# zju3dv/OnePose_Plus_Plus

Measured on AMD Instinct MI355X. Metric: query images/sec (2D-3D match fwd) at 512x512 img x 5k pts, higher is better.
Workload: dtype f32 (operands as exact bf16 triples, f32 accumulate)

## Files before the change

### onepose_plus_plus_amd/csrc/enc_layer64.hip

```cpp
#include <stdlib.h>

#include <type_traits>

#include "enc_frag.h"

namespace {

constexpr int R64 = 64, C = 256, NW = 8, NT = 512, D = 32;
constexpr int SA = a_stride_bytes(C);
constexpr int SS = C + 4;
constexpr int OFF_S = R64 * SA, OFF_Z = OFF_S + 32 * SS * 4;
constexpr size_t kLds64 = OFF_Z + 1024;

__global__ __launch_bounds__(NT) void enc_layer64_kernel(const OppEncChain a) {
  extern __shared__ __attribute__((aligned(16))) char smem[];
  char* A = smem;
  float* S = reinterpret_cast<float*>(smem + OFF_S);
  float* z_sh = reinterpret_cast<float*>(smem + OFF_Z);

  const int tid = threadIdx.x, lane = tid & 63;
  const int wave = __builtin_amdgcn_readfirstlane(tid >> 6);
  const int half = lane >> 5, l31 = lane & 31;

  const int chunks0 = (a.len0 + R64 - 1) / R64;
  const int stream = (int)blockIdx.x >= chunks0 ? 1 : 0;
  const int cidx = stream ? blockIdx.x - chunks0 : blockIdx.x;
  const int seg_len = stream ? a.len1 : a.len0;
  const int row0 = (stream ? a.len0 : 0) + cidx * R64;
  const int nrows = min(R64, seg_len - cidx * R64);
  const float* qrows = (stream && a.q1 != nullptr) ? a.q1 + (size_t)(cidx * R64) * a.ldq : a.q + (size_t)row0 * a.ldq;

  const char* a_lane = A + l31 * SA + half * 48;
  auto gemm = [&](auto ntile_c, auto depth_c, auto s0_c, auto s1_c, auto ks_c, const void* wf, int t0, f32x16 (&acc)[2][decltype(ntile_c)::value]) {
    constexpr int NTILE = decltype(ntile_c)::value, DEPTH = decltype(depth_c)::value;
    constexpr int S0 = decltype(s0_c)::value, S1 = decltype(s1_c)::value, KS = decltype(ks_c)::value;
    constexpr int NSTEP = S1 - S0;
    const __amdgpu_buffer_rsrc_t rsrc = __builtin_amdgcn_make_buffer_rsrc(const_cast<void*>(wf), 0, 0x7fffffff, 0x00020000);
    const int voff = lane * 16;
    u32x4 bq[DEPTH][NTILE][3];
    u32x4 af[2][2][3];
    auto load_b = [&](int s, int slot) {
#pragma unroll
      for (int j = 0; j < NTILE; ++j)
#pragma unroll
        for (int p = 0; p < 3; ++p)
          bq[slot][j][p] = __builtin_amdgcn_raw_buffer_load_b128(rsrc, voff, (((t0 + j) * KS + S0 + s) * 3 + p) * 1024, 0);
    };
    auto load_a = [&](int s, int slot) {
#pragma unroll
      for (int i = 0; i < 2; ++i)
#pragma unroll
        for (int q = 0; q < 3; ++q) af[slot][i][q] = *reinterpret_cast<const u32x4*>(a_lane + i * 32 * SA + s * 96 + q * 16);
    };
#pragma unroll
    for (int s = 0; s < DEPTH && s < NSTEP; ++s) load_b(s, s);
    load_a(0, 0);
    __builtin_amdgcn_sched_barrier(0);
    constexpr int PA[6] = {2, 0, 1, 1, 0, 0};
    constexpr int PB[6] = {0, 2, 1, 0, 1, 0};
#pragma unroll
    for (int s = 0; s < NSTEP; ++s) {
      if (s + 1 < NSTEP) load_a(s + 1, (s + 1) & 1);
#pragma unroll
      for (int pr = 0; pr < 6; ++pr)
#pragma unroll
        for (int i = 0; i < 2; ++i)
#pragma unroll
          for (int j = 0; j < NTILE; ++j)
            acc[i][j] = __builtin_amdgcn_mfma_f32_32x32x16_bf16(__builtin_bit_cast(bf16x8, af[s & 1][i][PA[pr]]),
                                                                 __builtin_bit_cast(bf16x8, bq[s % DEPTH][j][PB[pr]]), acc[i][j], 0, 0, 0);
      if (s + DEPTH < NSTEP) load_b(s + DEPTH, s % DEPTH);
      __builtin_amdgcn_sched_barrier(0);
    }
  };
  auto ic = [](auto v) { return v; };
  (void)ic;
  auto stage = [&](const f32x16& t, int col0, bool relu) {
#pragma unroll
    for (int r = 0; r < 16; ++r) {
      const int row = (r & 3) + 8 * (r >> 2) + 4 * half;
      float v = t[r];
      if (relu) v = v < 0.f ? 0.f : v;
      S[row * SS + col0 + l31] = v;
    }
  };
  auto split_staged = [&](int rb, int g0) {
#pragma unroll
    for (int i = 0; i < 32 * (C / 8) / NT; ++i) {
      const int p = tid + i * NT;
      const int r = p / (C / 8), g = p - r * (C / 8);
      const float4* s4 = reinterpret_cast<const float4*>(S + r * SS + g * 8);
      split8_store(s4[0], s4[1], A + (rb + r) * SA + (g0 + g) * 48);
    }
  };
  typedef float vec_t __attribute__((ext_vector_type(4)));
  auto layernorm_rows = [&](const float* gamma, const float* beta, float eps, auto mode_c, int rb) {
    constexpr int MODE = decltype(mode_c)::value;
    const vec_t gmv = *reinterpret_cast<const vec_t*>(gamma + lane * 4);
    const vec_t btv = *reinterpret_cast<const vec_t*>(beta + lane * 4);
    constexpr int RPW = 32 / NW;
    float v[RPW][4], sm[RPW], mean[RPW], rstd[RPW];
#pragma unroll
    for (int r = 0; r < RPW; ++r) {
      const vec_t t = *reinterpret_cast<const vec_t*>(S + (wave * RPW + r) * SS + lane * 4);
      sm[r] = 0.f;
#pragma unroll
      for (int i = 0; i < 4; ++i) {
        v[r][i] = t[i];
        sm[r] += t[i];
      }
    }
#pragma unroll
    for (int r = 0; r < RPW; ++r) sm[r] = opp_wave_sum_dpp(sm[r]);
#pragma unroll
    for (int r = 0; r < RPW; ++r) {
      mean[r] = sm[r] / (float)C;
      sm[r] = 0.f;
#pragma unroll
      for (int i = 0; i < 4; ++i) {
        const float d = v[r][i] - mean[r];
        sm[r] = opp_ln_sq_acc(d, sm[r]);
      }
    }
#pragma unroll
    for (int r = 0; r < RPW; ++r) sm[r] = opp_wave_sum_dpp(sm[r]);
#pragma unroll
    for (int r = 0; r < RPW; ++r) rstd[r] = 1.0f / sqrtf(sm[r] / (float)C + eps);
#pragma unroll
    for (int r = 0; r < RPW; ++r) {
      const int lr = rb + wave * RPW + r;
      float y[4];
#pragma unroll
      for (int i = 0; i < 4; ++i) y[i] = opp_ln_affine(v[r][i], mean[r], rstd[r], gmv[i], btv[i]);
      if constexpr (MODE != 0) {
        if (lr < nrows) {
          const vec_t xr = *reinterpret_cast<const vec_t*>(a.X + (size_t)(row0 + lr) * a.ldx + lane * 4);
          vec_t o;
#pragma unroll
          for (int i = 0; i < 4; ++i) o[i] = xr[i] + y[i];
          *reinterpret_cast<vec_t*>(a.out + (size_t)(row0 + lr) * a.ldo + lane * 4) = o;
#pragma unroll
          for (int i = 0; i < 4; ++i) y[i] = o[i];
        } else {
#pragma unroll
          for (int i = 0; i < 4; ++i) y[i] = 0.f;
        }
      }
      if constexpr (MODE != 1) {
        char* g = A + lr * SA + ((lane * 4) >> 3) * 48 + ((lane * 4) & 7) * 2;
#pragma unroll
        for (int i = 0; i < 4; i += 2) {
          unsigned hi, mid, lo;
          split2(y[i], y[i + 1], hi, mid, lo);
          *reinterpret_cast<unsigned*>(g + i * 2) = hi;
          *reinterpret_cast<unsigned*>(g + 16 + i * 2) = mid;
          *reinterpret_cast<unsigned*>(g + 32 + i * 2) = lo;
        }
      }
    }
  };
  auto zero2 = [](auto& acc) {
#pragma unroll
    for (auto& row : acc)
#pragma unroll
      for (auto& t : row)
#pragma unroll
        for (int r = 0; r < 16; ++r) t[r] = 0.f;
  };
  using I0 = std::integral_constant<int, 0>;
  using I1 = std::integral_constant<int, 1>;
  using I2 = std::integral_constant<int, 2>;
  using I3 = std::integral_constant<int, 3>;
  using I4 = std::integral_constant<int, 4>;
  using I16 = std::integral_constant<int, 16>;
  using I32 = std::integral_constant<int, 32>;

#pragma unroll
  for (int i = 0; i < R64 * (C / 8) / NT; ++i) {
    const int p = tid + i * NT;
    const int r = p / (C / 8), g = p - r * (C / 8);
    float4 v0 = make_float4(0.f, 0.f, 0.f, 0.f), v1 = v0;
    if (r < nrows) {
      const float4* s4 = reinterpret_cast<const float4*>(a.X + (size_t)(row0 + r) * a.ldx + g * 8);
      v0 = s4[0];
      v1 = s4[1];
    }
    split8_store(v0, v1, A + r * SA + g * 48);
  }
  const int src = a.cross ? 1 - stream : stream;
  const float src_len = (float)(src ? a.len1 : a.len0);
  const float* kvp = (src && a.kv1 != nullptr) ? a.kv1 : a.kv + (size_t)src * (C * D);
  const float* ksp = (src && a.ks1 != nullptr) ? a.ks1 : a.ks + (size_t)src * C;
  const int h = wave;
  float bk[16];
#pragma unroll
  for (int i = 0; i < 16; ++i) bk[i] = kvp[(h * D + 2 * i + half) * D + l31];
  __syncthreads();
  f32x16 hid[2][2];
  zero2(hid);
  gemm(I2{}, I3{}, I0{}, I16{}, I32{}, a.w1, wave * 2, hid);
  __syncthreads();

  constexpr int QS = 258;
  float* qsh = S;
#pragma unroll
  for (int rh = 0; rh < 2; ++rh) {
#pragma unroll
    for (int i = 0; i < 32 * (C / 4) / NT; ++i) {
      const int e = tid + i * NT;
      const int r = e / (C / 4), c4 = e - r * (C / 4);
      float4 q = make_float4(0.f, 0.f, 0.f, 0.f);
      if (rh * 32 + r < nrows) q = *reinterpret_cast<const float4*>(qrows + (size_t)(rh * 32 + r) * a.ldq + c4 * 4);
      float2* dst = reinterpret_cast<float2*>(qsh + r * QS + c4 * 4);
      dst[0] = make_float2(q.x, q.y);
      dst[1] = make_float2(q.z, q.w);
    }
    __syncthreads();
    if (tid < 8 * 32) {
      const int tok = tid & 31, hh = tid >> 5;
      const float* q = qsh + tok * QS + hh * D;
      const float* k = ksp + hh * D;
      float den = 0.f;
#pragma unroll
      for (int d = 0; d < D; ++d) den = fmaf(q[d], k[d], den);
      z_sh[hh * 32 + tok] = 1.0f / (den + a.eps_attn);
    }
    f32x16 num;
#pragma unroll
    for (int r = 0; r < 16; ++r) num[r] = 0.f;
#pragma unroll
    for (int i = 0; i < 16; ++i) num = __builtin_amdgcn_mfma_f32_32x32x2f32(qsh[l31 * QS + h * D + 2 * i + half], bk[i], num, 0, 0, 0);
    __syncthreads();
    {
      char* col = A + (h * 4 + (l31 >> 3)) * 48 + (l31 & 7) * 2;
#pragma unroll
      for (int r = 0; r < 16; ++r) {
        const int row = (r & 3) + 8 * (r >> 2) + 4 * half;
        const float v = (num[r] * z_sh[h * 32 + row]) * src_len;
        unsigned hi, mid, lo;
        split2(v, 0.f, hi, mid, lo);
        char* d = col + (rh * 32 + row) * SA;
        *reinterpret_cast<unsigned short*>(d) = (unsigned short)hi;
        *reinterpret_cast<unsigned short*>(d + 16) = (unsigned short)mid;
        *reinterpret_cast<unsigned short*>(d + 32) = (unsigned short)lo;
      }
    }
    __syncthreads();
  }

  {
    f32x16 acc[2][1];
    zero2(acc);
    gemm(I1{}, I4{}, I0{}, I16{}, I16{}, a.wm, wave, acc);
    __syncthreads();
#pragma unroll
    for (int rh = 0; rh < 2; ++rh) {
      stage(acc[rh][0], wave * 32, false);
      __syncthreads();
      layernorm_rows(a.g1, a.b1, a.eps_ln, I0{}, rh * 32);
      __syncthreads();
    }
  }

  gemm(I2{}, I3{}, I16{}, I32{}, I32{}, a.w1, wave * 2, hid);
  __syncthreads();

  f32x16 out[2][1];
  zero2(out);
#pragma unroll
  for (int kh = 0; kh < 2; ++kh) {
#pragma unroll
    for (int rh = 0; rh < 2; ++rh) {
      if (wave / (NW / 2) == kh) {
        const int c0 = (wave - kh * (NW / 2)) * 64;
        stage(hid[rh][0], c0, true);
        stage(hid[rh][1], c0 + 32, true);
      }
      __syncthreads();
      split_staged(rh * 32, 0);
      __syncthreads();
    }
    if (kh == 0) gemm(I1{}, I4{}, I0{}, I16{}, I32{}, a.w2, wave, out);
    else gemm(I1{}, I4{}, I16{}, I32{}, I32{}, a.w2, wave, out);
    __syncthreads();
  }

  const bool fold = a.wq_next != nullptr;
#pragma unroll
  for (int rh = 0; rh < 2; ++rh) {
    stage(out[rh][0], wave * 32, false);
    __syncthreads();
    if (fold) layernorm_rows(a.g2, a.b2, a.eps_ln, I2{}, rh * 32);
    else layernorm_rows(a.g2, a.b2, a.eps_ln, I1{}, rh * 32);
    __syncthreads();
  }
  if (!fold) return;

  float* qdst = (stream && a.qkv_out1 != nullptr) ? a.qkv_out1 + (size_t)(cidx * R64) * (3 * C) : a.qkv_out + (size_t)row0 * (3 * C);
  const float vdiv = (float)seg_len;
  auto store_qkv = [&](const f32x16& t, int rb, int tile) {
    const int col = tile * 32 + l31;
#pragma unroll
    for (int r = 0; r < 16; ++r) {
      const int row = rb + (r & 3) + 8 * (r >> 2) + 4 * half;
      if (row < nrows) {
        float v = t[r];
        if (col < 2 * C) v = v > 0.f ? v + 1.f : __expf(v);
        else v = v / vdiv;
        if (stream == 0 && a.qmask != nullptr) v *= a.qmask[row0 + row];
        qdst[(size_t)row * (3 * C) + col] = v;
      }
    }
  };
  {
    f32x16 acc[2][2];
    zero2(acc);
    gemm(I2{}, I3{}, I0{}, I16{}, I16{}, a.wq_next, wave * 3, acc);
#pragma unroll
    for (int i = 0; i < 2; ++i)
#pragma unroll
      for (int j = 0; j < 2; ++j) store_qkv(acc[i][j], i * 32, wave * 3 + j);
  }
  {
    f32x16 acc[2][1];
    zero2(acc);
    gemm(I1{}, I4{}, I0{}, I16{}, I16{}, a.wq_next, wave * 3 + 2, acc);
#pragma unroll
    for (int i = 0; i < 2; ++i) store_qkv(acc[i][0], i * 32, wave * 3 + 2);
  }
}

}

int opp_enc_layer64(const OppEncChain& a, hipStream_t stream) {
  OPP_CHECK_ARG(a.C == 256 && a.apply && a.X && a.out && a.q && a.kv && a.ks && a.wm && a.w1 && a.w2 && a.g1 && a.b1 && a.g2 && a.b2,
                "enc_layer64: coarse level (C = 256) with the fused attention apply only");
  OPP_CHECK_ARG(a.len0 >= 0 && a.len1 >= 0 && a.len0 + a.len1 > 0, "enc_layer64: empty token set");
  auto al16 = [](const void* p) { return (reinterpret_cast<uintptr_t>(p) & 15) == 0; };
  OPP_CHECK_ARG(al16(a.X) && al16(a.out) && al16(a.q) && a.ldx % 4 == 0 && a.ldo % 4 == 0 && a.ldq % 4 == 0 && al16(a.g1) && al16(a.b1) &&
                    al16(a.g2) && al16(a.b2) && al16(a.wm) && al16(a.w1) && al16(a.w2) && al16(a.q1), "enc_layer64: operands must be 16-byte aligned");
  OPP_CHECK_ARG(a.wq_next == nullptr || (a.qkv_out != nullptr && al16(a.wq_next)), "enc_layer64: folded projection needs its output buffer");
  static OppLdsOnce lds_once;
  opp_lds_opt_in(reinterpret_cast<const void*>(enc_layer64_kernel), kLds64, lds_once);
  const int tiles = opp_cdiv(a.len0, R64) + opp_cdiv(a.len1, R64);
  OppProfScope prof(OPP_PROF_ENC_CHAIN, stream, 2.0 * (double)(a.len0 + a.len1) * ((a.wq_next ? 10.0 : 7.0) * C * C + 32.0 * C));
  hipLaunchKernelGGL(enc_layer64_kernel, dim3(tiles), dim3(NT), kLds64, stream, a);
  OPP_CHECK_LAUNCH("enc_layer64_kernel");
  return OPP_OK;
}
```

### onepose_plus_plus_amd/csrc/gemm_mfma.hip

```cpp
#include <stdlib.h>

#include <mutex>
#include <type_traits>

#include <vector>

#include "opp_internal.h"

typedef float f32x16 __attribute__((ext_vector_type(16)));
typedef _Float16 f16x8 __attribute__((ext_vector_type(8)));
typedef __bf16 bf16x8 __attribute__((ext_vector_type(8)));
typedef __bf16 bf16x2 __attribute__((ext_vector_type(2)));
typedef float f32x2 __attribute__((ext_vector_type(2)));

namespace {

constexpr int lds_stride(int prec) { return prec == OPP_PREC_BF16X3 ? 52 : 36; }

__device__ __forceinline__ void opp_split4_b3(const float4 v, uint2& hi, uint2& mid, uint2& lo) {
  auto lvl = [](float a, float b, float& ra, float& rb) -> unsigned {
    const f32x2 t = {a, b};
    const unsigned p = __builtin_bit_cast(unsigned, __builtin_convertvector(t, bf16x2));
    ra = a - __uint_as_float(p << 16);
    rb = b - __uint_as_float(p & 0xffff0000u);
// ... 1522 lines not shown
    const int nkc = g.K / 32;
    const size_t need = (size_t)kSplits * g.M * g.ldc;
    const bool by_shape = splitk_by_shape(g);
    if ((g.splitk_force > 0 || (g.splitk_force < 0 && by_shape)) && nkc >= kSplits && g.splitk_ws_floats >= need && need < (1ull << 31)) {
      OppGemm gs = g;
      gs.C = g.splitk_ws;
      gs.C3 = nullptr;
      gs.k_splits = kSplits;
      gs.k_chunks_per_split = opp_cdiv(nkc, kSplits);
      gs.split_stride = (size_t)g.M * g.ldc;
      gs.bias = nullptr;
      gs.res_mode = OPP_RES_NONE;
      gs.R = nullptr;
      gs.act = OPP_ACT_NONE;
      gs.splitk_ws = nullptr;
      OPP_TRY(opp_gemm_launch_cfg(gs, 25, stream));
      const size_t n4 = (size_t)g.M * g.ldc / 4;
      const int blocks = (int)((n4 + 255) / 256 < 2048 ? (n4 + 255) / 256 : 2048);
      OppProfScope prof_epi(OPP_PROF_SPLITK_EPILOGUE, stream, (double)(kSplits + 1 + (g.res_mode == OPP_RES_DIRECT ? 1 : 0)) * (double)g.M * g.ldc * 4.0);
      hipLaunchKernelGGL(splitk_epilogue_kernel, dim3(blocks), dim3(256), 0, stream, reinterpret_cast<const float4*>(g.splitk_ws), kSplits, n4, n4, g.ldc / 4,
                         reinterpret_cast<const float4*>(g.bias), g.res_mode == OPP_RES_DIRECT ? reinterpret_cast<const float4*>(g.R) : nullptr, g.act,
                         reinterpret_cast<float4*>(g.C), g.C3, g.ld3);
      OPP_CHECK_LAUNCH("splitk_epilogue_kernel");
      return OPP_OK;
    }
  }
  const bool auto_cfg = cfg < 0;
  if (cfg < 0) cfg = choose_tile(g);
  OPP_CHECK_ARG(g.stat_rowmax == nullptr || (g.prec == OPP_PREC_BF16X3 ? (cfg == 25 || cfg == 20) : cfg == 0),
                "gemm: fused softmax statistics need the 128x128 tile (config 0; bf16x3: config 25, or 20 = 256x128)");
  if (g.ln_gamma != nullptr) {
    if (auto_cfg || (cfg != 30 && cfg != 26)) cfg = g.n_store == 256 ? 30 : 26;
    auto al = [](const void* p) { return (reinterpret_cast<uintptr_t>(p) & 15) == 0; };
    OPP_CHECK_ARG(g.ln_beta && ((cfg == 30 && g.n_store == 256) || (cfg == 26 && g.n_store == 128)) && g.N == g.n_store && !g.bias &&
                      g.act == OPP_ACT_NONE && g.res_mode == OPP_RES_NONE && g.ldc % 4 == 0 && al(g.C) && al(g.ln_gamma) &&
                      al(g.ln_beta) && (!g.ln_res || (al(g.ln_res) && g.ln_ldres % 4 == 0)),
                  "gemm: fused LayerNorm needs a 256- or 128-column output, no bias/activation/residual mode, aligned operands");
  }
  OppProfScope prof_scope(g.conv && g.k_splits > 1 ? (int)OPP_PROF_CONV_SPLITK : opp_prof_gemm_symbol(cfg, g.conv ? 1 : (g.stat_rowmax ? 2 : 0)), stream,
                          g.alg_flops > 0.0 ? g.alg_flops : 2.0 * (double)g.M * (double)g.N * (double)g.K);
  int rc;
  switch (cfg) {
    case 0: rc = launch_cfg<128, 128, 2, 2>(g, stream); break;
    case 1: rc = launch_cfg<64, 128, 2, 2>(g, stream); break;
    case 2: rc = launch_cfg<64, 64, 2, 2>(g, stream); break;
    case 10: rc = launch_cfg<128, 128, 2, 2, 3>(g, stream); break;
    case 11: rc = launch_cfg<128, 128, 2, 2, 4>(g, stream); break;
    case 20: rc = launch_cfg<256, 128, 4, 2>(g, stream); break;
    case 22:
      rc = conv208(g) ? launch_cfg<128, 224, 2, 4>(g, stream) : launch_cfg<128, 256, 2, 4>(g, stream);
      break;
    case 24: rc = launch_cfg<128, 192, 4, 2>(g, stream); break;
    case 25: rc = launch_cfg<128, 128, 4, 2>(g, stream); break;
    case 27:
      if (g.prec != OPP_PREC_BF16X3 || g.n_store > 224 || (g.n_real > 208 && g.n_real != g.n_store)) {
        opp_set_error("gemm: tile config 27 (128 x 224) is a bf16x3 tile for outputs of <= 208 real and <= 224 stored columns");
        rc = OPP_ERR_UNSUPPORTED;
      } else if (g.conv && (g.a_split || g.k_splits > 1)) {
        rc = launch_cfg<128, 256, 2, 4>(g, stream);
      } else if (g.conv) {
        rc = launch_cfg<128, 224, 2, 4>(g, stream);
      } else {
        rc = launch_cfg<128, 224, 4, 2>(g, stream);
      }
      break;
    case 26: rc = launch_cfg<64, 128, 2, 4>(g, stream); break;
    case 30: rc = launch_cfg<64, 256, 2, 4>(g, stream); break;
    default:
#ifdef OPP_TUNING
      rc = launch_tuning_cfg(g, cfg, stream);
#else
      opp_set_error("gemm: unknown tile config %d", cfg);
      rc = OPP_ERR_INVALID;
#endif
      break;
  }
  return rc;
}

extern "C" int opp_debug_timestamps(void* buf) {
#ifdef OPP_TUNING
  g_dbg_ts = static_cast<unsigned long long*>(buf);
  opp_gemm_ss_debug_timestamps(buf, getenv("OPP_SS_TS_MODE") ? atoi(getenv("OPP_SS_TS_MODE")) : 0);
  return OPP_OK;
#else
  (void)buf;
  opp_set_error("opp_debug_timestamps: library built without -DOPP_TUNING");
  return OPP_ERR_UNSUPPORTED;
#endif
}

int opp_gemm_launch(const OppGemm& g, hipStream_t stream) { return opp_gemm_launch_cfg(g, -1, stream); }

int opp_gemm_choose_tile(const OppGemm& g) {
  int cfg = choose_tile(g);
  if (g.conv && g.prec == OPP_PREC_BF16X3 && splitk_by_shape(g) && g.K / 32 >= 4) cfg = 1000 + 25;
  return cfg;
}
```

### onepose_plus_plus_amd/csrc/opp_internal.h

```cpp
#pragma once
#include "opp_common.h"

enum {
  OPP_PROF_FIRST_NON_GEMM = 1000,
  OPP_PROF_LINATTN_KV = 1000,
  OPP_PROF_LINATTN_APPLY = 1001,
  OPP_PROF_CONF = 1002,
  OPP_PROF_FINE = 1003,
  OPP_PROF_LINATTN_SMALL = 1004,
  OPP_PROF_FINE_GATHER = 1005,
  OPP_PROF_FINE_HEAD = 1006,
  OPP_PROF_FOCAL_FWD = 1007,
  OPP_PROF_FOCAL_BWD = 1008,
  OPP_PROF_ENC_CHAIN = 1009,
  OPP_PROF_SCORE_SWEEP1 = 1010,
  OPP_PROF_SCORE_SWEEP2 = 1011,
  OPP_PROF_CONV_WGRAD = 1013,
  OPP_PROF_CONV_SPLITK = 1014,
  OPP_PROF_CONV_TAIL = 1017,
  OPP_PROF_LINATTN_REDUCE = 1016,
  OPP_PROF_SPLITK_EPILOGUE = 1015,
  OPP_PROF_SCORE_SS = 1012,
};
inline int opp_prof_gemm_symbol(int tile_cfg, int kind) { return kind * 256 + tile_cfg; }
struct OppProfScope {
  OppProfScope(int symbol, hipStream_t stream, double work);
  ~OppProfScope();
  OppProfScope(const OppProfScope&) = delete;
  OppProfScope& operator=(const OppProfScope&) = delete;

 private:
  hipStream_t stream_;
  long long slot_ = -1;
};

int opp_layernorm(const float* x, int ldx, const float* gamma, const float* beta, const float* res, int ldres,
                  float* out, int ldo, int rows, int C, float eps, hipStream_t stream);
int opp_linattn_chunks(int seg_len);
int opp_linattn_kv(const float* k, const float* v, int ld, int n_seg, int seg_len, int C, int D, float* kv_out,
                   float* ks_out, float* scratch, hipStream_t stream);
int opp_linattn_apply(const float* q, int ldq, const float* kv, const float* ks, float* out, int ldo, int n_seg,
                      int seg_len, int src_len, int C, int D, float eps, hipStream_t stream);
size_t opp_linattn_pair_scratch_floats(int len0, int len1);
int opp_linattn_kv_pair(const float* qkv, int ld, int len0, int len1, float* kv, float* ks, float* scratch,
                        hipStream_t stream);
size_t opp_focal_loss_ws_bytes(size_t n);
int opp_focal_loss_fwd(const float* conf, const short* gt, const float* weight, size_t n, float alpha, float gamma, double* sums,
                       void* ws, size_t ws_bytes, hipStream_t stream);
int opp_focal_loss_bwd(const float* conf, const short* gt, const float* weight, size_t n, float alpha, float gamma,
                       const float* scales, float* grad, hipStream_t stream);
int opp_focal_loss_fwd_ex(const float* conf, const void* gt, int gt_kind, const float* weight, const float* mask0, const float* mask1, int N, int L,
                          size_t n, float alpha, float gamma, double* sums, void* ws, size_t ws_bytes, hipStream_t stream);
int opp_focal_loss_bwd_ex(const float* conf, const void* gt, int gt_kind, const float* weight, const float* mask0, const float* mask1, int N, int L,
                          size_t n, float alpha, float gamma, const float* scales, float* grad, hipStream_t stream);
size_t opp_dual_softmax_bwd_ws_bytes(int B, int N, int L);
int opp_dual_softmax_bwd(const float* g, const float* sim, const float* lse_row, const float* lse_col, int B, int N, int L, float* ds,
                         void* ws, size_t ws_bytes, hipStream_t stream);
bool opp_linattn_small_ok(int len0, int len1, int C, int D);
int opp_full_attention_run(const float* qkv, int n_seg, int len0, int len1, int C, int nhead, int cross, int prec, float* msg,
                           hipStream_t stream);
int opp_linattn_small_pair(const float* qkv, int ld, int n_seg, int len0, int len1, int cross, float* out, int ldo, int C, int D,
                           float eps, hipStream_t stream);
int opp_linattn_apply_pair(const float* qkv, int ld, const float* kv, const float* ks, int cross, float* out, int ldo,
                           int len0, int len1, float eps, hipStream_t stream);
struct OppEncChain {
  int C = 256;
  const float* X = nullptr;
  int ldx = 0;
  float* out = nullptr;
  int ldo = 0;
  int len0 = 0, len1 = 0;
  const float* msg = nullptr;
  int ldm = 0;
  int apply = 0;
  const float* q = nullptr;
  int ldq = 0;
  const float* kv = nullptr;
  const float* ks = nullptr;
  const float* q1 = nullptr;
  const float* kv1 = nullptr;
  const float* ks1 = nullptr;
  const void* wq_next = nullptr;
  float* qkv_out = nullptr;
  float* qkv_out1 = nullptr;
  const float* qmask = nullptr;
  int cross = 0;
  float eps_attn = 1e-6f;
  const void* wm = nullptr;
  const void* w1 = nullptr;
  const void* w2 = nullptr;
  const float *g1 = nullptr, *b1 = nullptr, *g2 = nullptr, *b2 = nullptr;
  float eps_ln = 1e-5f;
};
size_t opp_frag_b3_bytes(int N, int K);
int opp_pack_frag_b3(const float* w, int N, int K, void* out, hipStream_t stream);
bool opp_enc_chain_ok(int C, int nhead, bool apply);
int opp_enc_chain(const OppEncChain& a, hipStream_t stream);
int opp_enc_layer64(const OppEncChain& a, hipStream_t stream);
enum { OPP_SS_STATS = 1, OPP_SS_CONF = 2, OPP_SS_STATS_STORE = 3 };
struct OppGemmSS {
  const void* A = nullptr;
  const void* B = nullptr;
  int lda = 0, ldb = 0;
  int M = 0, N = 0, K = 0;
  int mode = OPP_SS_STATS;
  float out_mul = 1.f, out_div = 1.f;
  const float* row_mask = nullptr;
  float* stat_rowmax = nullptr;
  float* stat_rowsum = nullptr;
  float* stat_colmax = nullptr;
  float* stat_colsum = nullptr;
  const float* rstat_max = nullptr;
  const float* rstat_sum = nullptr;
  const float* cstat_max = nullptr;
  const float* cstat_sum = nullptr;
  float* C = nullptr;
  int ldc = 0;
  float* part_best = nullptr;
  int* part_arg = nullptr;
  int* part_ties = nullptr;
  float* part_rowmax = nullptr;
  int a_bytes = 0, b_bytes = 0, vec_store = 0;
  int delay = 0;
  unsigned long long* dbg_ts = nullptr;
};
void opp_gemm_ss_debug_timestamps(void* buf, int mode);
int opp_gemm_ss_tile_rows();
int opp_gemm_ss_tile_cols();
int opp_gemm_ss(const OppGemmSS& g, hipStream_t stream);
size_t opp_linear_bwd_ws_bytes(int M, int N, int K, int prec);
int opp_linear_bwd(const float* dY, const float* X, const float* W, int M, int N, int K, float* dX, float* dW, int accumulate_dw, int prec,
                   void* ws, size_t ws_bytes, hipStream_t stream);
size_t opp_linattn_train_ws_bytes(int B, int L, int S, int H, int D);
int opp_linattn_train_fwd(const float* q, const float* k, const float* v, const float* q_mask, const float* kv_mask, int B, int L, int S, int H, int D,
                          float eps, float* out, float* kv, float* ks, void* ws, size_t ws_bytes, hipStream_t stream);
int opp_linattn_train_bwd(const float* q, const float* k, const float* v, const float* q_mask, const float* kv_mask, const float* kv, const float* ks,
                          const float* grad_out, int B, int L, int S, int H, int D, float eps, float* gq, float* gk, float* gv, void* ws,
                          size_t ws_bytes, hipStream_t stream);
bool opp_stem_direct_ok(int cout, int prec);
int opp_stem_direct(const float* img, int H, int W, const float* wsplit, const float* bias, float* out, int ldc, hipStream_t stream, void* out3 = nullptr,
                    int ld3 = 0);
size_t opp_conv_tail_weight_floats(int cin_pad, int ks);
int opp_pack_conv_tail(const float* w, const float* scale, int cout, int cin, int ks, int n0, int cin_pad, float* wt, hipStream_t stream);
int opp_conv_tail(const OppGemm& g, const float* wt, int n0, int ncols, hipStream_t stream);
int opp_fold_bn(const float* gamma, const float* beta, const float* mean, const float* var, float eps, int c,
                int c_pad, float* scale, float* shift, hipStream_t stream);
int opp_pack_conv(const float* w, const float* scale, int cout, int cin, int ks, int cout_pad, int cin_pad,
                  float* out, hipStream_t stream);
int opp_pack_stem(const float* w, const float* scale, int cout, float* out, hipStream_t stream);
int opp_stem_im2col(const float* img, int B, int H, int W, float* col, hipStream_t stream);
int opp_h2_split(const float* in, float* out, size_t n, float* scale2, hipStream_t stream);
int opp_b3_split(const float* in, float* out, size_t n, hipStream_t stream);
int opp_add(const float* a, const float* b, float* out, size_t n, hipStream_t stream);
int opp_add_cat(const float* a, const float* b, size_t na, const float* c, size_t nc, float* out, hipStream_t stream);
int opp_transpose(const float* in, float* out, int batch, int R, int Cc, hipStream_t stream);
size_t opp_bn_train_scratch_bytes(int rows, int ld);
int opp_bn_train(const float* y, int rows, int ld, int C, const float* gamma, const float* beta, float eps, const float* res,
                 int act, float* out, float* stat_out, void* scratch, hipStream_t stream, float* save_mean = nullptr, float* save_invstd = nullptr);
size_t opp_conv_geo_entries(int P);
int opp_conv_geo(int B, int Ho, int Wo, int Hin, int Win, int ks, int stride, int pad, void* geo, hipStream_t stream);
size_t opp_conv_wgrad_ws_bytes(int P, int cout_pad, int cin_pad, int ks);
int opp_conv_wgrad(const float* dY, int ldy, const float* X, int ldx, size_t x_pixels, const void* geo, int P, int Win, int ks, int cout, int cin,
                   float* dW, int accumulate, void* ws, size_t ws_bytes, hipStream_t stream);
int opp_conv_flip_transpose(const float* w, int cout, int cin, int ks, float* out, hipStream_t stream);
int opp_conv_dilate2(const float* dy, int B, int Ho, int Wo, int ld, float* z, hipStream_t stream);
size_t opp_bn_bwd_scratch_bytes(int rows, int ld);
int opp_bn_backward(const float* dy, const float* y, const float* raw, int rows, int ld, int C, int act, const float* gamma, const float* mean,
                    const float* invstd, float* draw, float* dres, float* dgamma, float* dbeta, int accumulate, void* scratch, hipStream_t stream);
int opp_upsample2x_backward(const float* g, int B, int Hr, int Wr, int ld, float* dr, int accumulate, hipStream_t stream);
int opp_ln_forward(const float* x, const float* gamma, const float* beta, const float* res, int rows, int C, float eps, float* y, float* mean,
                   float* rstd, hipStream_t stream);
size_t opp_ln_backward_ws_bytes(int rows, int C);
int opp_ln_backward(const float* g, const float* x, const float* gamma, const float* mean, const float* rstd, int rows, int C, float* dx,
                    float* dgamma, float* dbeta, void* ws, size_t ws_bytes, hipStream_t stream);
size_t opp_lse_ws_bytes(int B, int N, int L);
int opp_dual_softmax_lse(const float* S, int B, int N, int L, float* lse_row, float* lse_col, float* conf, void* ws, size_t ws_bytes,
                         hipStream_t stream);
int opp_fine_gather_batch(const float* feat, int Hf, int Wf, int C, const long long* b_ids, const long long* j_ids, int M, int wc, int stride, int Wwin,
                          float* win, hipStream_t stream);
int opp_fine_scatter_batch(const float* gwin, int B, int Hf, int Wf, int C, const long long* b_ids, const long long* j_ids, int M, int wc, int stride,
                           int Wwin, float* dfeat, hipStream_t stream);
// ... 32 lines not shown
```

Measured before the change: 559.1.

## Pipeline weight prefetch across stages in fused 64-row encoder layer kernel

Moves the weight fragment ring into a struct so the next GEMM's B-fragments are primed during the tail of the previous GEMM. Query rows, residual X rows and the ks/qmask vectors are loaded early and overlapped with MFMA work. The attention denominator is computed per wave with a shuffle instead of a shared z buffer, and hidden activations are split straight to LDS without the S staging pass. Several __syncthreads are removed. Debug timestamp instrumentation is added behind OPP_TUNING. The cost is higher register pressure from the extra in-flight prefetches.

```diff
diff --git a/onepose_plus_plus_amd/csrc/enc_layer64.hip b/onepose_plus_plus_amd/csrc/enc_layer64.hip
--- a/onepose_plus_plus_amd/csrc/enc_layer64.hip
+++ b/onepose_plus_plus_amd/csrc/enc_layer64.hip
@@ -9,18 +9,71 @@
 constexpr int R64 = 64, C = 256, NW = 8, NT = 512, D = 32;
 constexpr int SA = a_stride_bytes(C);
 constexpr int SS = C + 4;
-constexpr int OFF_S = R64 * SA, OFF_Z = OFF_S + 32 * SS * 4;
-constexpr size_t kLds64 = OFF_Z + 1024;
-
-__global__ __launch_bounds__(NT) void enc_layer64_kernel(const OppEncChain a) {
+constexpr int OFF_S = R64 * SA, OFF_K = OFF_S + 32 * SS * 4, OFF_M = OFF_K + C * 4;
+constexpr size_t kLds64 = OFF_M + R64 * 4;
+constexpr int kStamps = 9, kTsStride = 16;
+#ifdef OPP_TUNING
+constexpr int kTsMaxTiles = 512, kTsLaunches = 16;
+#endif
+
+template <int NTILE_, int DEPTH_, int S0_, int S1_, int KS_>
+struct WRing {
+  static constexpr int NTILE = NTILE_, DEPTH = DEPTH_, S0 = S0_, NSTEP = S1_ - S0_, KS = KS_;
+  __amdgpu_buffer_rsrc_t rsrc;
+  int t0;
+  u32x4 bq[DEPTH][NTILE][3];
+  __device__ __forceinline__ void load(int s, int slot, int voff) {
+#pragma unroll
+    for (int j = 0; j < NTILE; ++j)
+#pragma unroll
+      for (int p = 0; p < 3; ++p)
+        bq[slot][j][p] = __builtin_amdgcn_raw_buffer_load_b128(rsrc, voff, (((t0 + j) * KS + S0 + s) * 3 + p) * 1024, 0);
+  }
+  __device__ __forceinline__ void prime(const void* wf, int tile0, int voff) {
+    rsrc = __builtin_amdgcn_make_buffer_rsrc(const_cast<void*>(wf), 0, 0x7fffffff, 0x00020000);
+    t0 = tile0;
+#pragma unroll
+    for (int s = 0; s < DEPTH && s < NSTEP; ++s) load(s, s, voff);
+  }
+};
+
+__device__ __forceinline__ void store_split16(char* d, float v) {
+  unsigned hi, mid, lo;
+  split2(v, 0.f, hi, mid, lo);
+  *reinterpret_cast<unsigned short*>(d) = (unsigned short)hi;
+  *reinterpret_cast<unsigned short*>(d + 16) = (unsigned short)mid;
+  *reinterpret_cast<unsigned short*>(d + 32) = (unsigned short)lo;
+}
+
+template <bool TS>
+__device__ __forceinline__ void enc_layer64_body(const OppEncChain& a, unsigned long long* ts) {
   extern __shared__ __attribute__((aligned(16))) char smem[];
   char* A = smem;
   float* S = reinterpret_cast<float*>(smem + OFF_S);
-  float* z_sh = reinterpret_cast<float*>(smem + OFF_Z);
+  float* ks_sh = reinterpret_cast<float*>(smem + OFF_K);
+  float* qm_sh = reinterpret_cast<float*>(smem + OFF_M);
 
   const int tid = threadIdx.x, lane = tid & 63;
   const int wave = __builtin_amdgcn_readfirstlane(tid >> 6);
   const int half = lane >> 5, l31 = lane & 31;
+  unsigned long long st[kStamps];
+  auto stamp = [&](int k) {
+    if constexpr (TS) {
+      __builtin_amdgcn_sched_barrier(0);
+      unsigned long long t;
+      asm volatile("s_memtime %0\n\ts_waitcnt lgkmcnt(0)" : "=s"(t)::"memory");
+      st[k] = t;
+      __builtin_amdgcn_sched_barrier(0);
+    }
+  };
+  auto flush_stamps = [&]() {
+    if constexpr (TS) {
+      if (tid == 0)
+#pragma unroll
+        for (int k = 0; k < kStamps; ++k) ts[(size_t)blockIdx.x * kTsStride + k] = st[k];
+    }
+  };
+  stamp(0);
 
   const int chunks0 = (a.len0 + R64 - 1) / R64;
   const int stream = (int)blockIdx.x >= chunks0 ? 1 : 0;
@@ -29,37 +82,30 @@
   const int row0 = (stream ? a.len0 : 0) + cidx * R64;
   const int nrows = min(R64, seg_len - cidx * R64);
   const float* qrows = (stream && a.q1 != nullptr) ? a.q1 + (size_t)(cidx * R64) * a.ldq : a.q + (size_t)row0 * a.ldq;
+  const int voff = lane * 16;
 
   const char* a_lane = A + l31 * SA + half * 48;
-  auto gemm = [&](auto ntile_c, auto depth_c, auto s0_c, auto s1_c, auto ks_c, const void* wf, int t0, f32x16 (&acc)[2][decltype(ntile_c)::value]) {
-    constexpr int NTILE = decltype(ntile_c)::value, DEPTH = decltype(depth_c)::value;
-    constexpr int S0 = decltype(s0_c)::value, S1 = decltype(s1_c)::value, KS = decltype(ks_c)::value;
-    constexpr int NSTEP = S1 - S0;
-    const __amdgpu_buffer_rsrc_t rsrc = __builtin_amdgcn_make_buffer_rsrc(const_cast<void*>(wf), 0, 0x7fffffff, 0x00020000);
-    const int voff = lane * 16;
-    u32x4 bq[DEPTH][NTILE][3];
+  auto run = [&](auto& ring, auto& acc, auto&& tail) {
+    using R = std::remove_reference_t<decltype(ring)>;
+    constexpr int NTILE = R::NTILE, DEPTH = R::DEPTH, NSTEP = R::NSTEP;
+    constexpr int TAIL = NSTEP >= 2 ? NSTEP - 2 : 0;
     u32x4 af[2][2][3];
-    auto load_b = [&](int s, int slot) {
-#pragma unroll
-      for (int j = 0; j < NTILE; ++j)
-#pragma unroll
-        for (int p = 0; p < 3; ++p)
-          bq[slot][j][p] = __builtin_amdgcn_raw_buffer_load_b128(rsrc, voff, (((t0 + j) * KS + S0 + s) * 3 + p) * 1024, 0);
-    };
     auto load_a = [&](int s, int slot) {
 #pragma unroll
       for (int i = 0; i < 2; ++i)
 #pragma unroll
         for (int q = 0; q < 3; ++q) af[slot][i][q] = *reinterpret_cast<const u32x4*>(a_lane + i * 32 * SA + s * 96 + q * 16);
     };
-#pragma unroll
-    for (int s = 0; s < DEPTH && s < NSTEP; ++s) load_b(s, s);
     load_a(0, 0);
     __builtin_amdgcn_sched_barrier(0);
     constexpr int PA[6] = {2, 0, 1, 1, 0, 0};
     constexpr int PB[6] = {0, 2, 1, 0, 1, 0};
 #pragma unroll
     for (int s = 0; s < NSTEP; ++s) {
+      if (s == TAIL) {
+        tail();
+        __builtin_amdgcn_sched_barrier(0);
+      }
       if (s + 1 < NSTEP) load_a(s + 1, (s + 1) & 1);
 #pragma unroll
       for (int pr = 0; pr < 6; ++pr)
@@ -68,37 +114,25 @@
 #pragma unroll
           for (int j = 0; j < NTILE; ++j)
             acc[i][j] = __builtin_amdgcn_mfma_f32_32x32x16_bf16(__builtin_bit_cast(bf16x8, af[s & 1][i][PA[pr]]),
-                                                                 __builtin_bit_cast(bf16x8, bq[s % DEPTH][j][PB[pr]]), acc[i][j], 0, 0, 0);
-      if (s + DEPTH < NSTEP) load_b(s + DEPTH, s % DEPTH);
+                                                                 __builtin_bit_cast(bf16x8, ring.bq[s % DEPTH][j][PB[pr]]), acc[i][j], 0, 0, 0);
+      if (s + DEPTH < NSTEP) ring.load(s + DEPTH, s % DEPTH, voff);
       __builtin_amdgcn_sched_barrier(0);
     }
   };
-  auto ic = [](auto v) { return v; };
-  (void)ic;
-  auto stage = [&](const f32x16& t, int col0, bool relu) {
+  auto no_tail = [] {};
+  auto stage = [&](const f32x16& t, int col0) {
 #pragma unroll
     for (int r = 0; r < 16; ++r) {
       const int row = (r & 3) + 8 * (r >> 2) + 4 * half;
-      float v = t[r];
-      if (relu) v = v < 0.f ? 0.f : v;
-      S[row * SS + col0 + l31] = v;
-    }
-  };
-  auto split_staged = [&](int rb, int g0) {
-#pragma unroll
-    for (int i = 0; i < 32 * (C / 8) / NT; ++i) {
-      const int p = tid + i * NT;
-      const int r = p / (C / 8), g = p - r * (C / 8);
-      const float4* s4 = reinterpret_cast<const float4*>(S + r * SS + g * 8);
-      split8_store(s4[0], s4[1], A + (rb + r) * SA + (g0 + g) * 48);
+      S[row * SS + col0 + l31] = t[r];
     }
   };
   typedef float vec_t __attribute__((ext_vector_type(4)));
-  auto layernorm_rows = [&](const float* gamma, const float* beta, float eps, auto mode_c, int rb) {
+  constexpr int RPW = 32 / NW;
+  auto layernorm_rows = [&](const float* gamma, const float* beta, float eps, auto mode_c, int rb, const vec_t (&xr)[RPW]) {
     constexpr int MODE = decltype(mode_c)::value;
     const vec_t gmv = *reinterpret_cast<const vec_t*>(gamma + lane * 4);
     const vec_t btv = *reinterpret_cast<const vec_t*>(beta + lane * 4);
-    constexpr int RPW = 32 / NW;
     float v[RPW][4], sm[RPW], mean[RPW], rstd[RPW];
 #pragma unroll
     for (int r = 0; r < RPW; ++r) {
@@ -134,10 +168,9 @@
       for (int i = 0; i < 4; ++i) y[i] = opp_ln_affine(v[r][i], mean[r], rstd[r], gmv[i], btv[i]);
       if constexpr (MODE != 0) {
         if (lr < nrows) {
-          const vec_t xr = *reinterpret_cast<const vec_t*>(a.X + (size_t)(row0 + lr) * a.ldx + lane * 4);
           vec_t o;
 #pragma unroll
-          for (int i = 0; i < 4; ++i) o[i] = xr[i] + y[i];
+          for (int i = 0; i < 4; ++i) o[i] = xr[r][i] + y[i];
           *reinterpret_cast<vec_t*>(a.out + (size_t)(row0 + lr) * a.ldo + lane * 4) = o;
 #pragma unroll
           for (int i = 0; i < 4; ++i) y[i] = o[i];
@@ -159,6 +192,7 @@
       }
     }
   };
+  const vec_t no_x[RPW] = {};
   auto zero2 = [](auto& acc) {
 #pragma unroll
     for (auto& row : acc)
@@ -170,11 +204,16 @@
   using I0 = std::integral_constant<int, 0>;
   using I1 = std::integral_constant<int, 1>;
   using I2 = std::integral_constant<int, 2>;
-  using I3 = std::integral_constant<int, 3>;
-  using I4 = std::integral_constant<int, 4>;
-  using I16 = std::integral_constant<int, 16>;
-  using I32 = std::integral_constant<int, 32>;
-
+
+  WRing<2, 3, 0, 16, 32> w1a;
+  w1a.prime(a.w1, wave * 2, voff);
+  const int src = a.cross ? 1 - stream : stream;
+  const float src_len = (float)(src ? a.len1 : a.len0);
+  const float* kvp = (src && a.kv1 != nullptr) ? a.kv1 : a.kv + (size_t)src * (C * D);
+  const float* ksp = (src && a.ks1 != nullptr) ? a.ks1 : a.ks + (size_t)src * C;
+  if (tid < C / 4) reinterpret_cast<float4*>(ks_sh)[tid] = reinterpret_cast<const float4*>(ksp)[tid];
+  const bool use_mask = stream == 0 && a.qmask != nullptr && a.wq_next != nullptr;
+  if (use_mask && tid < nrows) qm_sh[tid] = a.qmask[row0 + tid];
 #pragma unroll
   for (int i = 0; i < R64 * (C / 8) / NT; ++i) {
     const int p = tid + i * NT;
@@ -187,135 +226,175 @@
     }
     split8_store(v0, v1, A + r * SA + g * 48);
   }
-  const int src = a.cross ? 1 - stream : stream;
-  const float src_len = (float)(src ? a.len1 : a.len0);
-  const float* kvp = (src && a.kv1 != nullptr) ? a.kv1 : a.kv + (size_t)src * (C * D);
-  const float* ksp = (src && a.ks1 != nullptr) ? a.ks1 : a.ks + (size_t)src * C;
   const int h = wave;
   float bk[16];
 #pragma unroll
   for (int i = 0; i < 16; ++i) bk[i] = kvp[(h * D + 2 * i + half) * D + l31];
   __syncthreads();
+  stamp(1);
   f32x16 hid[2][2];
   zero2(hid);
-  gemm(I2{}, I3{}, I0{}, I16{}, I32{}, a.w1, wave * 2, hid);
-  __syncthreads();
-
   constexpr int QS = 258;
   float* qsh = S;
-#pragma unroll
-  for (int rh = 0; rh < 2; ++rh) {
+  float4 qr[2][32 * (C / 4) / NT];
+  auto load_q = [&](int rh) {
 #pragma unroll
     for (int i = 0; i < 32 * (C / 4) / NT; ++i) {
       const int e = tid + i * NT;
       const int r = e / (C / 4), c4 = e - r * (C / 4);
-      float4 q = make_float4(0.f, 0.f, 0.f, 0.f);
-      if (rh * 32 + r < nrows) q = *reinterpret_cast<const float4*>(qrows + (size_t)(rh * 32 + r) * a.ldq + c4 * 4);
+      qr[rh][i] = rh * 32 + r < nrows ? *reinterpret_cast<const float4*>(qrows + (size_t)(rh * 32 + r) * a.ldq + c4 * 4) : make_float4(0.f, 0.f, 0.f, 0.f);
+    }
+  };
+  auto put_q = [&](int rh) {
+#pragma unroll
+    for (int i = 0; i < 32 * (C / 4) / NT; ++i) {
+      const int e = tid + i * NT;
+      const int r = e / (C / 4), c4 = e - r * (C / 4);
       float2* dst = reinterpret_cast<float2*>(qsh + r * QS + c4 * 4);
-      dst[0] = make_float2(q.x, q.y);
-      dst[1] = make_float2(q.z, q.w);
-    }
+      dst[0] = make_float2(qr[rh][i].x, qr[rh][i].y);
+      dst[1] = make_float2(qr[rh][i].z, qr[rh][i].w);
+    }
+  };
+  run(w1a, hid, [&] { load_q(0); });
+  stamp(2);
+
+  WRing<1, 4, 0, 16, 16> wmr;
+  wmr.prime(a.wm, wave, voff);
+  load_q(1);
+  put_q(0);
+#pragma unroll
+  for (int rh = 0; rh < 2; ++rh) {
     __syncthreads();
-    if (tid < 8 * 32) {
-      const int tok = tid & 31, hh = tid >> 5;
-      const float* q = qsh + tok * QS + hh * D;
-      const float* k = ksp + hh * D;
-      float den = 0.f;
-#pragma unroll
-      for (int d = 0; d < D; ++d) den = fmaf(q[d], k[d], den);
-      z_sh[hh * 32 + tok] = 1.0f / (den + a.eps_attn);
-    }
+    const float* q = qsh + l31 * QS + h * D;
+    float den = 0.f;
+#pragma unroll
+    for (int d = 0; d < D; ++d) den = fmaf(q[d], ks_sh[h * D + d], den);
+    const float z = 1.0f / (den + a.eps_attn);
     f32x16 num;
 #pragma unroll
     for (int r = 0; r < 16; ++r) num[r] = 0.f;
 #pragma unroll
     for (int i = 0; i < 16; ++i) num = __builtin_amdgcn_mfma_f32_32x32x2f32(qsh[l31 * QS + h * D + 2 * i + half], bk[i], num, 0, 0, 0);
-    __syncthreads();
-    {
-      char* col = A + (h * 4 + (l31 >> 3)) * 48 + (l31 & 7) * 2;
-#pragma unroll
-      for (int r = 0; r < 16; ++r) {
-        const int row = (r & 3) + 8 * (r >> 2) + 4 * half;
-        const float v = (num[r] * z_sh[h * 32 + row]) * src_len;
-        unsigned hi, mid, lo;
-        split2(v, 0.f, hi, mid, lo);
-        char* d = col + (rh * 32 + row) * SA;
-        *reinterpret_cast<unsigned short*>(d) = (unsigned short)hi;
-        *reinterpret_cast<unsigned short*>(d + 16) = (unsigned short)mid;
-        *reinterpret_cast<unsigned short*>(d + 32) = (unsigned short)lo;
-      }
-    }
-    __syncthreads();
-  }
-
+    if (rh == 0) {
+      __syncthreads();
+      put_q(1);
+    }
+    char* col = A + (h * 4 + (l31 >> 3)) * 48 + (l31 & 7) * 2;
+#pragma unroll
+    for (int r = 0; r < 16; ++r) {
+      const int row = (r & 3) + 8 * (r >> 2) + 4 * half;
+      const float v = (num[r] * __shfl(z, row)) * src_len;
+      store_split16(col + (rh * 32 + row) * SA, v);
+    }
+  }
+  __syncthreads();
+  stamp(3);
+
+  WRing<2, 3, 16, 32, 32> w1b;
   {
     f32x16 acc[2][1];
     zero2(acc);
-    gemm(I1{}, I4{}, I0{}, I16{}, I16{}, a.wm, wave, acc);
-    __syncthreads();
+    run(wmr, acc, no_tail);
+    w1b.prime(a.w1, wave * 2, voff);
 #pragma unroll
     for (int rh = 0; rh < 2; ++rh) {
-      stage(acc[rh][0], wave * 32, false);
+      stage(acc[rh][0], wave * 32);
       __syncthreads();
-      layernorm_rows(a.g1, a.b1, a.eps_ln, I0{}, rh * 32);
+      layernorm_rows(a.g1, a.b1, a.eps_ln, I0{}, rh * 32, no_x);
       __syncthreads();
     }
   }
-
-  gemm(I2{}, I3{}, I16{}, I32{}, I32{}, a.w1, wave * 2, hid);
-  __syncthreads();
-
+  stamp(4);
+
+  WRing<1, 4, 0, 16, 32> w2a;
+  run(w1b, hid, [&] { w2a.prime(a.w2, wave, voff); });
+  __syncthreads();
+  stamp(5);
+
+  auto store_hidden = [&](int kh) {
+    if (wave / (NW / 2) == kh) {
+      const int c0 = (wave - kh * (NW / 2)) * 64;
+#pragma unroll
+      for (int j = 0; j < 2; ++j) {
+        const int k = c0 + j * 32 + l31;
+        char* col = A + (k >> 3) * 48 + (k & 7) * 2;
+#pragma unroll
+        for (int rh = 0; rh < 2; ++rh)
+#pragma unroll
+          for (int r = 0; r < 16; ++r) {
+            const int row = rh * 32 + (r & 3) + 8 * (r >> 2) + 4 * half;
+            float v = hid[rh][j][r];
+            v = v < 0.f ? 0.f : v;
+            store_split16(col + row * SA, v);
+          }
+      }
+    }
+  };
   f32x16 out[2][1];
   zero2(out);
-#pragma unroll
-  for (int kh = 0; kh < 2; ++kh) {
-#pragma unroll
-    for (int rh = 0; rh < 2; ++rh) {
-      if (wave / (NW / 2) == kh) {
-        const int c0 = (wave - kh * (NW / 2)) * 64;
-        stage(hid[rh][0], c0, true);
-        stage(hid[rh][1], c0 + 32, true);
-      }
-      __syncthreads();
-      split_staged(rh * 32, 0);
-      __syncthreads();
-    }
-    if (kh == 0) gemm(I1{}, I4{}, I0{}, I16{}, I32{}, a.w2, wave, out);
-    else gemm(I1{}, I4{}, I16{}, I32{}, I32{}, a.w2, wave, out);
+  store_hidden(0);
+  __syncthreads();
+  WRing<1, 4, 16, 32, 32> w2b;
+  run(w2a, out, [&] { w2b.prime(a.w2, wave, voff); });
+  __syncthreads();
+  store_hidden(1);
+  __syncthreads();
+  const bool fold = a.wq_next != nullptr;
+  vec_t xres[2][RPW];
+  WRing<2, 3, 0, 16, 16> wqa;
+  run(w2b, out, [&] {
+#pragma unroll
+    for (int rh = 0; rh < 2; ++rh)
+#pragma unroll
+      for (int r = 0; r < RPW; ++r) {
+        const int lr = rh * 32 + wave * RPW + r;
+        xres[rh][r] = lr < nrows ? *reinterpret_cast<const vec_t*>(a.X + (size_t)(row0 + lr) * a.ldx + lane * 4) : vec_t{};
+      }
+  });
+  if (fold) wqa.prime(a.wq_next, wave * 3, voff);
+  stamp(6);
+
+#pragma unroll
+  for (int rh = 0; rh < 2; ++rh) {
+    stage(out[rh][0], wave * 32);
     __syncthreads();
-  }
-
-  const bool fold = a.wq_next != nullptr;
-#pragma unroll
-  for (int rh = 0; rh < 2; ++rh) {
-    stage(out[rh][0], wave * 32, false);
+    if (fold) layernorm_rows(a.g2, a.b2, a.eps_ln, I2{}, rh * 32, xres[rh]);
+    else layernorm_rows(a.g2, a.b2, a.eps_ln, I1{}, rh * 32, xres[rh]);
     __syncthreads();
-    if (fold) layernorm_rows(a.g2, a.b2, a.eps_ln, I2{}, rh * 32);
-    else layernorm_rows(a.g2, a.b2, a.eps_ln, I1{}, rh * 32);
-    __syncthreads();
-  }
-  if (!fold) return;
+  }
+  stamp(7);
+  if (!fold) {
+    stamp(8);
+    flush_stamps();
+    return;
+  }
 
   float* qdst = (stream && a.qkv_out1 != nullptr) ? a.qkv_out1 + (size_t)(cidx * R64) * (3 * C) : a.qkv_out + (size_t)row0 * (3 * C);
   const float vdiv = (float)seg_len;
-  auto store_qkv = [&](const f32x16& t, int rb, int tile) {
+  auto store_qkv_as = [&](const f32x16& t, int rb, int tile, auto is_v_c) {
     const int col = tile * 32 + l31;
 #pragma unroll
     for (int r = 0; r < 16; ++r) {
       const int row = rb + (r & 3) + 8 * (r >> 2) + 4 * half;
       if (row < nrows) {
         float v = t[r];
-        if (col < 2 * C) v = v > 0.f ? v + 1.f : __expf(v);
+        if constexpr (!decltype(is_v_c)::value) v = v > 0.f ? v + 1.f : __expf(v);
         else v = v / vdiv;
-        if (stream == 0 && a.qmask != nullptr) v *= a.qmask[row0 + row];
+        if (use_mask) v *= qm_sh[row];
         qdst[(size_t)row * (3 * C) + col] = v;
       }
     }
   };
+  auto store_qkv = [&](const f32x16& t, int rb, int tile) {
+    if (tile * 32 < 2 * C) store_qkv_as(t, rb, tile, std::false_type{});
+    else store_qkv_as(t, rb, tile, std::true_type{});
+  };
+  WRing<1, 4, 0, 16, 16> wqb;
   {
     f32x16 acc[2][2];
     zero2(acc);
-    gemm(I2{}, I3{}, I0{}, I16{}, I16{}, a.wq_next, wave * 3, acc);
+    run(wqa, acc, no_tail);
+    wqb.prime(a.wq_next, wave * 3 + 2, voff);
 #pragma unroll
     for (int i = 0; i < 2; ++i)
 #pragma unroll
@@ -324,13 +403,29 @@
   {
     f32x16 acc[2][1];
     zero2(acc);
-    gemm(I1{}, I4{}, I0{}, I16{}, I16{}, a.wq_next, wave * 3 + 2, acc);
+    run(wqb, acc, no_tail);
 #pragma unroll
     for (int i = 0; i < 2; ++i) store_qkv(acc[i][0], i * 32, wave * 3 + 2);
   }
+  stamp(8);
+  flush_stamps();
 }
 
+__global__ __launch_bounds__(NT) void enc_layer64_kernel(const OppEncChain a) { enc_layer64_body<false>(a, nullptr); }
+#ifdef OPP_TUNING
+__global__ __launch_bounds__(NT) void enc_layer64_ts_kernel(const OppEncChain a, unsigned long long* ts) { enc_layer64_body<true>(a, ts); }
+unsigned long long* g_ts = nullptr;
+int g_ts_launch = 0;
+#endif
+
 }
+
+#ifdef OPP_TUNING
+void opp_enc_layer64_debug_timestamps(void* buf) {
+  g_ts = static_cast<unsigned long long*>(buf);
+  g_ts_launch = 0;
+}
+#endif
 
 int opp_enc_layer64(const OppEncChain& a, hipStream_t stream) {
   OPP_CHECK_ARG(a.C == 256 && a.apply && a.X && a.out && a.q && a.kv && a.ks && a.wm && a.w1 && a.w2 && a.g1 && a.b1 && a.g2 && a.b2,
@@ -341,9 +436,21 @@
                     al16(a.g2) && al16(a.b2) && al16(a.wm) && al16(a.w1) && al16(a.w2) && al16(a.q1), "enc_layer64: operands must be 16-byte aligned");
   OPP_CHECK_ARG(a.wq_next == nullptr || (a.qkv_out != nullptr && al16(a.wq_next)), "enc_layer64: folded projection needs its output buffer");
   static OppLdsOnce lds_once;
+#ifdef OPP_TUNING
+  static OppLdsOnce lds_once_ts;
+#endif
   opp_lds_opt_in(reinterpret_cast<const void*>(enc_layer64_kernel), kLds64, lds_once);
   const int tiles = opp_cdiv(a.len0, R64) + opp_cdiv(a.len1, R64);
   OppProfScope prof(OPP_PROF_ENC_CHAIN, stream, 2.0 * (double)(a.len0 + a.len1) * ((a.wq_next ? 10.0 : 7.0) * C * C + 32.0 * C));
+#ifdef OPP_TUNING
+  if (g_ts != nullptr && g_ts_launch < kTsLaunches && tiles <= kTsMaxTiles) {
+    opp_lds_opt_in(reinterpret_cast<const void*>(enc_layer64_ts_kernel), kLds64, lds_once_ts);
+    unsigned long long* ts = g_ts + (size_t)(g_ts_launch++) * kTsMaxTiles * kTsStride;
+    hipLaunchKernelGGL(enc_layer64_ts_kernel, dim3(tiles), dim3(NT), kLds64, stream, a, ts);
+    OPP_CHECK_LAUNCH("enc_layer64_ts_kernel");
+    return OPP_OK;
+  }
+#endif
   hipLaunchKernelGGL(enc_layer64_kernel, dim3(tiles), dim3(NT), kLds64, stream, a);
   OPP_CHECK_LAUNCH("enc_layer64_kernel");
   return OPP_OK;
diff --git a/onepose_plus_plus_amd/csrc/gemm_mfma.hip b/onepose_plus_plus_amd/csrc/gemm_mfma.hip
--- a/onepose_plus_plus_amd/csrc/gemm_mfma.hip
+++ b/onepose_plus_plus_amd/csrc/gemm_mfma.hip
@@ -1628,6 +1628,7 @@
 #ifdef OPP_TUNING
   g_dbg_ts = static_cast<unsigned long long*>(buf);
   opp_gemm_ss_debug_timestamps(buf, getenv("OPP_SS_TS_MODE") ? atoi(getenv("OPP_SS_TS_MODE")) : 0);
+  opp_enc_layer64_debug_timestamps(buf);
   return OPP_OK;
 #else
   (void)buf;
diff --git a/onepose_plus_plus_amd/csrc/opp_internal.h b/onepose_plus_plus_amd/csrc/opp_internal.h
--- a/onepose_plus_plus_amd/csrc/opp_internal.h
+++ b/onepose_plus_plus_amd/csrc/opp_internal.h
@@ -97,6 +97,7 @@
 bool opp_enc_chain_ok(int C, int nhead, bool apply);
 int opp_enc_chain(const OppEncChain& a, hipStream_t stream);
 int opp_enc_layer64(const OppEncChain& a, hipStream_t stream);
+void opp_enc_layer64_debug_timestamps(void* buf);
 enum { OPP_SS_STATS = 1, OPP_SS_CONF = 2, OPP_SS_STATS_STORE = 3 };
 struct OppGemmSS {
   const void* A = nullptr;
```

Measured after the change: 561.1, median of 6. Within noise of the previous version (+0.4%).
